# gitAugust/Aruco_Slam

Measured on AMD Instinct MI355X. Metric: frames/s (detect+pose+EKF) at 1280x720, 20 markers, 200 landmarks, higher is better.
Workload: dtype u8/f64; 1 GPU; cfg2: 1280x720 gray stream per GPU, 20 markers/frame in view, 200-landmark EKF (N=603), frames resident in HBM, detector {'polygonalApproxAccuracyRate': 0.03, 'doCornerRefinement': 1}; streams=1, ekf=True, asserted=every frame: 20 markers detected, 20 corrections fused, map_gather=none

## Files before the change

### aruco_slam_amd/csrc/capi.hip

```cpp
#include "common.h"
#include "detect.h"
#include "pose.h"
#include "ekf.h"
#include "win_plan.h"
#include "synth.h"
#include "../../include/aruco_slam_hip.h"
#include <string>
#include <vector>
#include <cfloat>
#include <fstream>
#include <sstream>
#include <cctype>
#include <cstdio>
#include <cstring>
#include <cstdlib>
#include <dlfcn.h>
#include <cstdio>
#include <cmath>
#include <algorithm>
#include <chrono>

using namespace aslam;

namespace {
// ... 117 lines not shown
    bool slam_gate_on = false;
    aslam_gate_params slam_gate_prm{};
    SlamGateArg slam_gate{};
    bool slam_gate_windows = false;
    bool umap_on = false;
    MapCov umap{};
    double* d_map_c = nullptr;
    TrackHealth* h_track_health = nullptr;

    bool win_enabled = true;
    int win_piece = kWinChainFrames;
    bool win_pieces = false;
    unsigned win_epoch = 0;
    bool win_no_early = false;
    bool win_next_split = false;
    struct Pending { bool active = false; int first = 0, count = 0, ev = 0; } pend;
    hipEvent_t ev_obs[2] = {nullptr, nullptr}, ev_idx = nullptr;
    hipStream_t stream_win = nullptr;
    hipEvent_t ev_win[64] = {};
    unsigned win_count = 0;
    unsigned ev_win_next = 0;
    int ev_obs_next = 0;
    bool ev_idx_set = false;
    ObsRaw* h_obs = nullptr;
    unsigned* h_nm = nullptr;
    WinFrame* h_win_frames = nullptr;
    PlanMirror mirror;
    bool mirror_dirty = true;
    int ekf_lo = 0, ekf_hi = 0;
    double last_timing[6] = {0, 0, 0, 0, 0, 0};
// ... 524 lines not shown
    if (c->init.cap_points_per_frame == 0) c->init.cap_points_per_frame = 1u << 19;
    c->max_batch = init->max_batch;
    c->nwaves = init->persistent_waves > 0 ? init->persistent_waves : 4096;
    if (init->persistent_waves <= 0) {
        const char* e = std::getenv("ASLAM_PERSISTENT_WAVES");
        if (e && std::atoi(e) > 0) c->nwaves = std::atoi(e);
    }
    c->sp.Q_k = init->Q_k; c->sp.R_x = init->R_x; c->sp.R_y = init->R_y; c->sp.R_theta = init->R_theta;
    c->sp.kl = init->kl; c->sp.kr = init->kr; c->sp.b = init->b; c->sp.marker_length = init->marker_length;
    c->sp.r2c_tx = init->r2c_t[0]; c->sp.r2c_ty = init->r2c_t[1];
    c->sp.useful_distance_threshold = init->useful_distance_threshold;

    c->win_enabled = std::getenv("ASLAM_NO_WINDOWS") == nullptr;
    c->win_no_early = std::getenv("ASLAM_WIN_NO_EARLY") != nullptr;
    c->win_next_split = std::getenv("ASLAM_WIN_NEXT_SPLIT") != nullptr;
    if (const char* e = std::getenv("ASLAM_WIN_PIECE")) { c->win_piece = std::min(kWinChainFrames, std::max(1, std::atoi(e))); c->win_pieces = true; }
    const int B = c->max_batch;
    const size_t px = (size_t)init->max_rows * init->max_cols;
    const size_t pitch = ((size_t)init->max_cols + 63) / 64 * 64;
    int prio_lo = 0, prio_hi = 0;
    hipDeviceGetStreamPriorityRange(&prio_lo, &prio_hi);
    bool ok = hipStreamCreateWithPriority(&c->stream, hipStreamNonBlocking, prio_lo) == hipSuccess;
    ok = ok && hipStreamCreateWithPriority(&c->stream_ekf, hipStreamNonBlocking, prio_hi) == hipSuccess;
    {
        hipDeviceProp_t prop{};
        const bool known = hipGetDeviceProperties(&prop, init->device_id) == hipSuccess && prop.multiProcessorCount == 256 &&
                           std::strncmp(prop.gcnArchName, "gfx950", 6) == 0;
        const int nxcd = 8, per_xcd = 32;
        const int res = init->ekf_reserved_cus_per_xcd == 0 ? (c->win_enabled ? 4 : 16) : init->ekf_reserved_cus_per_xcd;
        if (known && res > 0 && res < per_xcd) {
// ... 221 lines not shown
int win_steps(const aslam_ctx* c, int first_slot, int K) {
    int n = 0;
    for (int k = 0; k < K; k++) n += 1 + c->h_win_frames[first_slot + k].m;
    return n;
}

void enqueue_window_one(aslam_ctx* c, const WinOp& o, const WinDesc& wd) {
    hipStream_t sa = c->stream_ekf;
    WinDesc cw = wd;
    cw.first_slot = o.frame; cw.K = o.K; cw.piece = 0; cw.log0 = 0; cw.last = 1; cw.mu_out = 0;
    if (++c->win_epoch == 0) c->win_epoch = 1;
    cw.epoch = c->win_epoch;
    cw.nsteps = win_steps(c, o.frame, o.K);
    prof_begin(c, P_EKF_WIN_CHAIN, sa);
    const bool gated = gated_windows(c);
    launch_ekf_win_one(sa, c->ekf, c->sp, cw, c->d_obs, c->d_enc, gated ? &c->slam_gate : nullptr);
    prof_end(c);
    if (gated) {
        prof_begin(c, P_EKF_WIN_GATE_FINISH, sa);
        launch_ekf_win_gate_finish(sa, c->ekf, cw, c->slam_gate, c->d_obs);
        prof_end(c);
    }
}

int enqueue_window_pieces(aslam_ctx* c, const WinOp& o, const WinDesc& wd, hipEvent_t ev_prev_flush) {
    hipStream_t sa = c->stream_ekf;
    struct Piece { WinDesc sub; int nsteps; };
    std::vector<Piece> pieces;
    int log0 = 0, k0 = 0;
    for (int kn : win_piece_sizes(o.K, c->win_piece)) {
        Piece pc;
// ... 2643 lines not shown
```

### aruco_slam_amd/csrc/ekf.h

```cpp
#pragma once
#include "common.h"

namespace aslam {

constexpr int kIdTableSize = 1024;

struct PopRec {
    int id, index, action, det;
    double z[3];
    double r[3];
};
struct LastObs {
    int id, pad;
    double z[3];
};
struct UpdRec {
    int li, pad;
    double Gxm[18];
    double ze[3];
    double r[3];
};
struct MapRecord {
    int id, index;
    double x, y, theta;
// ... 220 lines not shown
    size_t stride;
    const int* robot_of_slot;
    RelocParams prm;
    const ObsRaw* obs;
    const unsigned* n_markers;
    int first, apply;
    RelocRecord* out;
    SlamRelocSeat* seat;
};
hipError_t slam_reloc_alloc(SlamRelocBufs& B, int slots);
void slam_reloc_free(SlamRelocBufs& B);
void launch_slam_reloc_solve(hipStream_t st, const SlamReloc& A, int count);
void launch_slam_reloc_seat(hipStream_t st, const SlamReloc& A, int count);
inline int ekf_win_tiles(int nS) { return nS <= 20 ? 4 : nS <= 41 ? 8 : 12; }
void launch_ekf_win_one(hipStream_t st, const EkfState& E, const SlamParams& sp, const WinDesc& wd, const ObsRaw* obs, const double* enc,
                        const SlamGateArg* gate = nullptr);
void launch_ekf_win_gate_finish(hipStream_t st, const EkfState& E, const WinDesc& wd, const SlamGateArg& gate, const ObsRaw* obs);
void launch_ekf_win_step(hipStream_t st, const EkfState& E, const SlamParams& sp, const WinDesc& wd, const ObsRaw* obs, const double* enc,
                         int s_piece, int s_log0, int s_nsteps, int q_piece, int q_log0, int q_nsteps);
void launch_ekf_win_gather(hipStream_t st, const EkfState& E, const WinDesc& wd);
void launch_ekf_win_next(hipStream_t st, const EkfState& E, const WinDesc& pv, const WinDesc& nx, bool split);
void launch_ekf_win_flush(hipStream_t st, const EkfState& E, const WinDesc& wd);

}
```

### aruco_slam_amd/csrc/ekf_window.hip

```cpp
#include "common.h"
#include "ekf.h"
#include "ekf_dev.h"
#include "ekf_slam_gate.h"
#include <cmath>
#include <cstdlib>
#include <algorithm>

namespace aslam {

constexpr int WBW = 8;
constexpr int kWinPubEvery = 4, kWinPubLag = 4;
#if defined(__HIP__)
constexpr unsigned long long kWinSpinTicks = 2000000;
#else
constexpr unsigned long long kWinSpinTicks = 6000000000ull;
#endif
__device__ __forceinline__ void win_fail(const EkfState& E, unsigned code) { atomicCAS(E.d_win_err, 0u, code); }
template <int NC> __device__ __forceinline__ void win_vmcnt_lag() {
    static_assert(kWinPubLag == 4 && NC >= 1 && NC <= 3, "the counts below are (3 NC + 1) kWinPubLag");
    static_assert((3 * NC + 1) * kWinPubLag <= 63, "vmcnt has six bits");
    if constexpr (NC == 1) ASLAM_VMCNT(16);
    else if constexpr (NC == 2) ASLAM_VMCNT(28);
    else ASLAM_VMCNT(40);
}

#ifdef ASLAM_WIN_STAMPS
#define WSTAMP(i) do { const long long t_ = clock64(); stamp_acc[i] += t_ - stamp_last; stamp_last = t_; } while (0)
#else
#define WSTAMP(i) do { } while (0)
#endif

__host__ __device__ inline int win_log_stride(int T) { return 3 * 16 * T + kWinHdr; }
__host__ __device__ inline int win_tlog_stride(int T) { return 8 * 16 * T; }
enum { WH_TYPE = 0, WH_POS = 1, WH_SI = 2, WH_ZE = 11, WH_C = 14, WH_S = 15, WH_G02 = 16, WH_G12 = 17, WH_A = 18, WH_B = 19, WH_D2 = 20, WH_ACC = 21 };
struct WinGate { static constexpr bool kOn = true; double gate_d2; };
template <class G> struct WinArg : WinDesc, G {};
static_assert(sizeof(WinArg<NoSlamGate>) == sizeof(WinDesc), "the ungated window argument is the window descriptor alone");
__host__ __device__ inline size_t wsm_P(int SPm, int par) { return (size_t)par * SPm * SPm; }
__host__ __device__ inline size_t wsm_LAM(int SPm, int par) { return (size_t)(2 + par) * SPm * SPm; }
__host__ __device__ inline size_t wsm_PSI(int SPm, int par) { return (size_t)(4 + par) * SPm * SPm; }
__host__ __device__ inline size_t wsm_psi(int SPm, int par) { return (size_t)6 * SPm * SPm + (size_t)par * SPm; }
__host__ __device__ inline size_t wsm_MU(int SPm, int par) { return (size_t)6 * SPm * SPm + (size_t)(2 + par) * SPm; }
__host__ __device__ inline size_t wsm_doubles(int SPm) { return (size_t)6 * SPm * SPm + (size_t)4 * SPm; }

// ... 55 lines not shown
        LastObs lo;
        lo.id = o.id; lo.pad = 0;
        const double nanv = __builtin_nan("");
        lo.z[0] = upd ? o.x : nanv; lo.z[1] = upd ? o.y : nanv; lo.z[2] = upd ? o.th : nanv;
        E.d_last[lane] = lo;
    }
    if (lane == 0) { *E.d_nlast = npop; *E.d_npop = npop; *E.d_m = fm; }
}

template <int T, bool ONE> struct WinChainLds {
    static constexpr int SP = 16 * T, SPP = SP + 16, KMAX = ONE ? kWinFrames : kWinPieceMax, NSMAX = KMAX * 64;
    double sA[2][4][SPP];
    double sB[2][4][SPP];
    double sPub[2][3][SPP];
    double sHdr[2][kWinHdr];
    double sRec[2][5][64];
#ifdef ASLAM_WIN_POSE_CHECK
    double sDbg[2][3][SPP];
#endif
    double sMu[SPP];
    int sS[SP];
    int sOff[KMAX + 1];
    unsigned char sPos[NSMAX], sIdx[NSMAX];
    unsigned char sDet[NSMAX];
    static constexpr int kGrown = 2 * 5 * 64 * (int)sizeof(double) - NSMAX;
};
template <bool GATED, class LDS> __device__ __forceinline__ double win_header_entry(const LDS& L, int j, int cb, int fpar, int lane) {
    double v = L.sHdr[cb][lane];
    const int pos = L.sPos[j];
    if (pos != 255) {
        const int a = L.sIdx[j];
        const int q = lane >= WH_ZE && lane < WH_ZE + 3 ? lane - WH_ZE : lane == WH_G02 ? 3 : lane == WH_G12 ? 4 : -1;
        if (q >= 0) v = L.sRec[fpar][q][a];
        if (!GATED && lane == WH_TYPE) v = 1.0;
        if (lane == WH_POS) v = (double)pos;
    }
    return v;
}
template <int T, int RW, bool ONE, class G>
__device__ void win_chain_role(const EkfState& E, const SlamParams& sp, const WinDesc& wd, const G& gate, const ObsRaw* __restrict__ obs,
                               const double* __restrict__ enc, unsigned char* smem) {
    static_assert(ONE || !G::kOn, "only the one-launch window is gated");
    constexpr int SP = 16 * T, SPP = SP + 16, NC = SP / 64;
    constexpr int NWK = (T + RW - 1) / RW, NT = (NWK + (ONE ? 2 : 1)) * 64;
    WinChainLds<T, ONE>& L = *reinterpret_cast<WinChainLds<T, ONE>*>(smem);
    auto& sA = L.sA; auto& sB = L.sB; auto& sPub = L.sPub; auto& sMu = L.sMu; auto& sS = L.sS; auto& sOff = L.sOff;
    auto& sPos = L.sPos; auto& sIdx = L.sIdx; auto& sDet = L.sDet;
    if (threadIdx.x >= NT) return;
    const int tid = threadIdx.x;
    const int nS = wd.nS, s = 3 + 3 * nS;
    const int ld = E.ld;
    const WinFrame* __restrict__ frames = E.d_win_frames;

    const int wave = tid >> 6, lane = tid & 63;
    const int li = lane & 15, lk = lane >> 4;
    for (int e = tid; e < SP; e += NT) sS[e] = e < s ? win_state_index(wd, e) : 0;
    for (int e = tid; e < 2 * 4 * SPP; e += NT) { (&sA[0][0][0])[e] = 0.0; (&sB[0][0][0])[e] = 0.0; }
// ... 139 lines not shown
            printf("worker %d T %d steps %d: barrier-wait %lld | B reads %lld A reads + products%s %lld publish %lld cycles per step\n", wave, T, NS, stamp_acc[0] / (NS + 1),
                   stamp_acc[1] / (NS + 1), ONE ? "" : " + log", stamp_acc[2] / (NS + 1), stamp_acc[3] / (NS + 1));
#endif
        double* Pout = E.d_win_small + wsm_P(E.win_sp_max, wd.wpar);
#pragma unroll
        for (int rr = 0; rr < RW; rr++)
#pragma unroll
            for (int t = 0; t < T; t++)
#pragma unroll
                for (int reg = 0; reg < 4; reg++)
                    if (T % RW == 0 || wave * RW + rr < T) Pout[(size_t)(16 * (wave * RW + rr) + lk + 4 * reg) * SP + 16 * t + li] = acc[rr][t][reg];
        return;
    }

    if (ONE && wave == NWK + 1) {
        ASLAM_LDS_BARRIER();
        win_last_frame(E, frames[wd.first_slot + wd.K - 1], obs + (size_t)(wd.first_slot + wd.K - 1) * kMarkerMax, sOff[wd.K] - sOff[wd.K - 1] - 1, lane);
#ifdef ASLAM_WIN_STAMPS
        long long stamp_acc[2] = {0, 0}, stamp_last = clock64();
#endif
        int fpar = 1;
        for (int j = -1; j < NS; j++) {
            WSTAMP(0);
            if (j > kWinPubLag && j % kWinPubEvery == 0 && lane == 0) win_signal(E.d_win_sync, wd.epoch, j - kWinPubLag);
            if (j >= 0) {
                const int cb = j & 1;
                double* const log = logbase + (size_t)j * win_log_stride(T);
#pragma unroll
                for (int k = 0; k < 3; k++)
#pragma unroll
                    for (int c = 0; c < NC; c++) st_wt(log + k * SP + lane + 64 * c, sA[cb][k][lane + 64 * c]);
                if (sPos[j] == 255) fpar ^= 1;
                if (lane < kWinHdr) st_wt(log + 3 * SP + lane, win_header_entry<G::kOn>(L, j, cb, fpar, lane));
                if ((j + 1) % kWinPubEvery == 0) win_vmcnt_lag<NC>();
            }
            WSTAMP(1);
            ASLAM_LDS_BARRIER();
        }
        ASLAM_VMCNT(0);
        if (lane == 0) win_signal(E.d_win_sync, wd.epoch, NS);
#ifdef ASLAM_WIN_STAMPS
        if (lane == 0) printf("logger T %d steps %d: barrier-wait %lld work %lld cycles per step\n", T, NS, stamp_acc[0] / (NS + 1), stamp_acc[1] / (NS + 1));
#endif
        return;
    }

#ifndef ASLAM_NO_SETPRIO
    __builtin_amdgcn_s_setprio(3);
#endif
    const double kl = sp.kl, kr = sp.kr, inv2b = 1.0 / (2 * sp.b), invb = 1 / sp.b, Qk = sp.Q_k;
    double* const muimg = E.d_win_small + wsm_MU(E.win_sp_max, wd.wpar);
    double mu[NC], pB[4][NC];
    double rp[3][NC];
#pragma unroll
    for (int c = 0; c < NC; c++) {
        const int col = lane + 64 * c;
        mu[c] = col >= s ? 0.0 : from_img ? muimg[col] : E.d_mu[sS[col]];
#pragma unroll
        for (int k = 0; k < 4; k++) pB[k][c] = 0.0;
#pragma unroll
        for (int q = 0; q < 3; q++) rp[q][c] = from_img ? Pimg[(size_t)q * SP + col] : col < s ? E.d_sigma[(size_t)sS[col] * ld + sS[q]] : 0.0;
    }
#ifdef ASLAM_WIN_POSE_CHECK
    double dmax = 0.0, dend = 0.0;
#endif
    double rze0 = 0, rze1 = 0, rze2 = 0, rR0 = 0, rR1 = 0, rR2 = 0, rg02 = 0, rg12 = 0;
    double cth = 1.0, sth = 0.0;
    int fk = -1, fm = 0, fa = 0, vpos = 0;
    bool prev_predict = false;
    bool dirty0 = false, dirty1 = false;
    ObsRaw nObs{};
    if (lane < sOff[1] - 1) nObs = obs[(size_t)wd.first_slot * kMarkerMax + sDet[1 + lane]];
    double e_wl, e_wr, e_dt;
    { const double* e = enc + (size_t)3 * wd.first_slot; e_wl = e[0]; e_wr = e[1]; e_dt = e[2]; }
    ASLAM_LDS_BARRIER();
#ifdef ASLAM_WIN_STAMPS
    long long stamp_acc[11] = {0, 0, 0, 0, 0, 0, 0, 0, 0, 0, 0}, stamp_last = clock64();
    int n_pred = 0;
#endif
    for (int j = -1; j < NS; j++) {
        const int n = j + 1;
        WSTAMP(0);
        if (n < NS) {
            const int nb = n & 1, pb = j & 1;
            const bool is_predict = fa == fm;
// ... 32 lines not shown
                    for (int c = 0; c < NC; c++) {
                        r[0][c] = fma(f[kk][0], pB[kk][c], r[0][c]); r[1][c] = fma(f[kk][1], pB[kk][c], r[1][c]); r[2][c] = fma(f[kk][2], pB[kk][c], r[2][c]);
                        r[3][c] = fma(f[kk][3], pB[kk][c], r[3][c]); r[4][c] = fma(f[kk][4], pB[kk][c], r[4][c]); r[5][c] = fma(f[kk][5], pB[kk][c], r[5][c]);
                    }
                }
            }
#pragma unroll
            for (int c = 0; c < NC; c++) { rp[0][c] = r[0][c]; rp[1][c] = r[1][c]; rp[2][c] = r[2][c]; }
            WSTAMP(1);
            double* const hdr = L.sHdr[nb];
            double A[4][NC], B[4][NC];
            if (is_predict) {
#ifdef ASLAM_WIN_STAMPS
                n_pred++;
#endif
                const int k = ++fk;
                const int slot = wd.first_slot + k;
                fm = ASLAM_WAVE_BCAST(sOff[k + 1] - sOff[k] - 1, 0); fa = 0;
                const double delta_sl = kl * (e_dt * e_wl), delta_sr = kr * (e_dt * e_wr);
                const double delta_theta = (delta_sr - delta_sl) * inv2b;
                const double delta_s = 0.5 * (delta_sr + delta_sl);
#pragma unroll
                for (int c = 0; c < NC; c++) sMu[lane + 64 * c] = mu[c];
                __builtin_amdgcn_wave_barrier();
                const double m0 = sMu[0], m1 = sMu[1], m2 = sMu[2];
#ifdef ASLAM_WIN_STAMPS
                asm volatile("s_waitcnt lgkmcnt(0)" ::: "memory");
                WSTAMP(8);
#endif
                double th = m2 + delta_theta;
// ... 9 lines not shown
                const double P22 = ASLAM_WAVE_BCAST(r[2][0], 2);
#pragma unroll
                for (int c = 0; c < NC; c++) {
                    const int col = lane + 64 * c;
                    const double u = col == 0 ? ua : col == 1 ? ub : 0.0;
                    const double w0 = col == 0 ? f * cm : col == 1 ? f * sm : col == 2 ? f * invb : 0.0;
                    const double w1 = col == 0 ? f * cm : col == 1 ? f * sm : col == 2 ? f * -invb : 0.0;
                    A[0][c] = u;                       B[0][c] = r[2][c];
                    A[1][c] = fma(P22, u, r[2][c]);    B[1][c] = u;
                    A[2][c] = su0 * w0;                B[2][c] = w0;
                    A[3][c] = su1 * w1;                B[3][c] = w1;
                    sA[nb][3][col] = A[3][c]; sB[nb][3][col] = B[3][c];
                }
                if (nb) dirty1 = true; else dirty0 = true;
                const double np0 = m0 + delta_s * cm, np1 = m1 + delta_s * sm;
                if (lane == 0) mu[0] = np0;
                if (lane == 1) mu[0] = np1;
                if (lane == 2) mu[0] = th;
                if (lane < fm) {
                    vpos = sPos[sOff[k] + 1 + lane];
                    const int q = 3 + 3 * vpos;
                    const double mx = sMu[q], my = sMu[q + 1], mth = sMu[q + 2];
                    const double gdx = mx - np0, gdy = my - np1;
                    double gdth = mth - th;
                    wrap1(gdth);
                    const double zh0 = gdx * cth + gdy * sth, zh1 = -gdx * sth + gdy * cth;
                    double z2 = nObs.th - gdth;
                    wrap1(z2);
                    rze0 = nObs.x - zh0; rze1 = nObs.y - zh1; rze2 = z2;
                    rg02 = -gdx * sth + gdy * cth; rg12 = -gdx * cth - gdy * sth;
                    rR0 = nObs.r[0]; rR1 = nObs.r[1]; rR2 = nObs.r[2];
                    double (&rec)[5][64] = L.sRec[k & 1];
                    rec[0][lane] = rze0; rec[1][lane] = rze1; rec[2][lane] = rze2; rec[3][lane] = rg02; rec[4][lane] = rg12;
                }
                __builtin_amdgcn_wave_barrier();
                WSTAMP(10);
                if constexpr (!ONE) {
                    if (wd.last && k == wd.K - 1) win_last_frame(E, frames[slot], obs + (size_t)slot * kMarkerMax, fm, lane);
                }
                if (k + 1 < wd.K) {
                    const int fmn = sOff[k + 2] - sOff[k + 1] - 1;
                    if (lane < fmn) nObs = obs[(size_t)(slot + 1) * kMarkerMax + sDet[sOff[k + 1] + 1 + lane]];
                    const double* e = enc + (size_t)3 * (slot + 1);
                    e_wl = e[0]; e_wr = e[1]; e_dt = e[2];
                }
                if (lane == 0) { hdr[WH_TYPE] = 0.0; hdr[WH_POS] = -1.0; hdr[WH_A] = ua; hdr[WH_B] = ub; hdr[WH_C] = cth; hdr[WH_S] = sth; }
                WSTAMP(2);
            } else {
// ... 23 lines not shown
                Sm[0] += R0; Sm[4] += R1; Sm[8] += R2;
                inv3_fast(Sm, Si);
                double d2 = 0.0;
                bool rejected = false;
                if constexpr (G::kOn) {
                    d2 = slam_gate_d2(Si, ze0, ze1, ze2);
                    rejected = gate.gate_d2 < HUGE_VAL && !(d2 <= gate.gate_d2);
                }
                WSTAMP(4);
#pragma unroll
                for (int c = 0; c < NC; c++) {
                    const double k0 = cc[0][c] * Si[0] + cc[1][c] * Si[3] + cc[2][c] * Si[6];
                    const double k1 = cc[0][c] * Si[1] + cc[1][c] * Si[4] + cc[2][c] * Si[7];
                    const double k2 = cc[0][c] * Si[2] + cc[1][c] * Si[5] + cc[2][c] * Si[8];
                    if constexpr (G::kOn) {
                        const double dm = k0 * ze0 + k1 * ze1 + k2 * ze2;
                        mu[c] = rejected ? mu[c] : mu[c] + dm;
                        A[0][c] = rejected ? 0.0 : -k0; A[1][c] = rejected ? 0.0 : -k1; A[2][c] = rejected ? 0.0 : -k2; A[3][c] = 0.0;
                    } else {
                        mu[c] += k0 * ze0 + k1 * ze1 + k2 * ze2;
                        A[0][c] = -k0; A[1][c] = -k1; A[2][c] = -k2; A[3][c] = 0.0;
                    }
                    B[0][c] = cc[0][c]; B[1][c] = cc[1][c]; B[2][c] = cc[2][c]; B[3][c] = 0.0;
                }
                if (nb ? dirty1 : dirty0) {
#pragma unroll
                    for (int c = 0; c < NC; c++) { sA[nb][3][lane + 64 * c] = 0.0; sB[nb][3][lane + 64 * c] = 0.0; }
                    if (nb) dirty1 = false; else dirty0 = false;
                }
                if (lane == 0) {
#pragma unroll
                    for (int q = 0; q < 9; q++) hdr[WH_SI + q] = Si[q];
                    if constexpr (G::kOn) { hdr[WH_TYPE] = rejected ? 2.0 : 1.0; hdr[WH_D2] = d2; hdr[WH_ACC] = rejected ? 0.0 : 1.0; }
                }
                WSTAMP(5);
            }
#pragma unroll
            for (int c = 0; c < NC; c++) {
                const int col = lane + 64 * c;
                sA[nb][0][col] = A[0][c]; sA[nb][1][col] = A[1][c]; sA[nb][2][col] = A[2][c];
                if (is_predict) { sB[nb][0][col] = B[0][c]; sB[nb][1][col] = B[1][c]; sB[nb][2][col] = B[2][c]; }
#pragma unroll
                for (int kk = 0; kk < 4; kk++) pB[kk][c] = B[kk][c];
            }
            prev_predict = is_predict;
            WSTAMP(6);
        }
        ASLAM_LDS_BARRIER();
    }
#ifdef ASLAM_WIN_STAMPS
    if (lane == 0 && (ONE || wd.piece == 1)) {
        const int nc = NS - n_pred;
        printf("prepare T %d steps %d (%d predict): barrier %lld | rows wait %lld correct %lld | predict path %lld (mean through LDS %lld sincos %lld operands + records %lld global loads, bookkeeping, header %lld) per predict | c %lld S+inv %lld Kt+hdr %lld per correction | operands+log %lld per step\n",
               T, NS, n_pred, stamp_acc[0] / (NS + 1), stamp_acc[7] / NS, stamp_acc[1] / NS, (stamp_acc[2] + stamp_acc[8] + stamp_acc[9] + stamp_acc[10]) / (n_pred ? n_pred : 1), stamp_acc[8] / (n_pred ? n_pred : 1),
               stamp_acc[9] / (n_pred ? n_pred : 1), stamp_acc[10] / (n_pred ? n_pred : 1), stamp_acc[2] / (n_pred ? n_pred : 1), stamp_acc[3] / (nc ? nc : 1), stamp_acc[4] / (nc ? nc : 1),
               stamp_acc[5] / (nc ? nc : 1), stamp_acc[6] / NS);
    }
#endif
#ifdef ASLAM_WIN_POSE_CHECK
    if (lane == 0) printf("pose-check T %d piece %d steps %d: max |prepare - accumulator| pose rows %.3e over the piece, %.3e at its end\n", T, wd.piece, NS, dmax, dend);
#endif
#pragma unroll
    for (int c = 0; c < NC; c++) {
        const int col = lane + 64 * c;
        if (col < s) { muimg[col] = mu[c]; if (wd.mu_out) E.d_mu[sS[col]] = mu[c]; }
    }
}

struct WinReplay { int piece, log0, nsteps, wpar; };
template <int T> struct WinScanLds {
    static constexpr int SP = 16 * T, REC = 3 * SP + kWinHdr;
    double sLam[SP][WBW + 1];
    double sRec[2][REC];
    double sT[2][4][WBW];
};
template <int T, bool ONE, bool GATED>
__device__ void win_scan_role(const EkfState& E, const WinReplay& wd, int b, unsigned epoch, int* sAvail, unsigned char* smem) {
    constexpr int SP = 16 * T, EPT = SP * WBW / 256, REC = 3 * SP + kWinHdr;
    constexpr int RPT = (REC + 191) / 192;
    WinScanLds<T>& L = *reinterpret_cast<WinScanLds<T>*>(smem);
// ... 183 lines not shown
            for (int reg = 0; reg < 4; reg++) Psi[(size_t)(16 * tr + lk + 4 * reg) * SP + 16 * tc + li] = acc[q][reg];
        }
    }
}

__device__ __forceinline__ int win_ticket(unsigned long long* w, unsigned epoch) {
    unsigned long long old = __hip_atomic_load((aslam_gu64*)w, __ATOMIC_RELAXED, __HIP_MEMORY_SCOPE_AGENT);
    for (;;) {
        const bool cur = (unsigned)(old >> 32) == epoch;
        const unsigned long long nw = cur ? old + 1 : ((unsigned long long)epoch << 32) | 1u;
        const unsigned long long prev = atomicCAS(w, old, nw);
        if (prev == old) return cur ? (int)(unsigned)old : 0;
        old = prev;
    }
}
template <int T, int RW, bool ONE, class G = NoSlamGate>
__global__ __launch_bounds__(((T + RW - 1) / RW + (ONE ? 2 : 1)) * 64 > 256 ? ((T + RW - 1) / RW + (ONE ? 2 : 1)) * 64 : 256)
void k_ekf_win_step(EkfState E, SlamParams sp, WinArg<G> wa, WinReplay rs, WinReplay rq, const ObsRaw* __restrict__ obs, const double* __restrict__ enc) {
    const WinDesc& wd = wa;
    constexpr size_t kLds = sizeof(WinChainLds<T, ONE>) > sizeof(WinScanLds<T>) ? sizeof(WinChainLds<T, ONE>) : sizeof(WinScanLds<T>);
    __shared__ __align__(16) unsigned char smem[kLds];
    __shared__ int sTicket, sAvail;
    constexpr int NSCAN = 16 * T / WBW;
    int bx = blockIdx.x;
    if constexpr (ONE) {
        if (threadIdx.x == 0) sTicket = win_ticket(E.d_win_sync + (size_t)kWinSyncLine * (kWinSyncCounters - 1), wd.epoch);
        __syncthreads();
        bx = sTicket;
    }
    if (bx == 0) { if (wd.K > 0) win_chain_role<T, RW, ONE, G>(E, sp, wd, static_cast<const G&>(wa), obs, enc, smem); }
    else if (bx <= NSCAN) { if (rs.nsteps > 0) win_scan_role<T, ONE, G::kOn>(E, rs, bx - 1, wd.epoch, &sAvail, smem); }
    else if (rq.nsteps > 0) win_psi_role<T, ONE, G::kOn>(E, rq, bx - 1 - NSCAN, wd.epoch, &sAvail);
}

constexpr int kWinFinishThreads = 1024;
__global__ __launch_bounds__(kWinFinishThreads) void k_ekf_win_gate_finish(EkfState E, WinDesc wd, GateState gs, const ObsRaw* __restrict__ obs) {
    constexpr int NW = kWinFinishThreads / 64;
    __shared__ double sD2[NW][64];
    __shared__ int sKind[NW][64], sFlag[NW][64], sId[NW][64];
    __shared__ int sOff[kWinFrames + 1], sAtt[kWinFrames], sAcc[kWinFrames];
    const int tid = threadIdx.x, wave = tid >> 6, lane = tid & 63;
    const int K = min(wd.K, kWinFrames);
    const WinFrame* __restrict__ frames = E.d_win_frames + wd.first_slot;
    const int ls = win_log_stride(wd.T), SP = 16 * wd.T;
    const double* __restrict__ hdr0 = E.d_win_log + (size_t)wd.log0 * ls + 3 * SP;
// ... 274 lines not shown
        for (int pc = 0; pc < SPp; pc += 64) {
            double bv[16];
#pragma unroll
            for (int g = 0; g < 16; g++) bv[g] = W[(size_t)(pc + 4 * g) * ld];
#pragma unroll
            for (int g = 0; g < 16; g++) acc = __builtin_amdgcn_mfma_f64_16x16x4f64(-sTt[pc + 4 * g + lk][li], pr == -1 ? bv[g] : 0.0, acc, 0, 0, 0);
        }
#pragma unroll
        for (int reg = 0; reg < 4; reg++) {
            const int c = c0 + lk + 4 * reg;
            if (pr == -1 && sPa[c] == -1) Pout[(size_t)r * SPn + c] = acc[reg];
        }
    }
}

template <int T, bool ONE, class K, class W> static void launch_step_kernel(K kernel, hipStream_t st, int nb, int nt, size_t static_lds, const EkfState& E, const SlamParams& sp,
                                                const W& wd, const WinReplay& rs, const WinReplay& rq, const ObsRaw* obs, const double* enc) {
    static const bool share = std::getenv("ASLAM_WIN_SHARE_CU") != nullptr;
    constexpr size_t cap = (size_t)24 * 1024 + WinChainLds<T, ONE>::kGrown;
    const size_t dyn = share ? 0 : (size_t)84 * 1024 - std::min(static_lds, cap);
    static bool attr_done = false;
    if (!attr_done && dyn > 0) {
        (void)hipFuncSetAttribute(reinterpret_cast<const void*>(kernel), hipFuncAttributeMaxDynamicSharedMemorySize, (int)dyn);
        attr_done = true;
    }
    hipLaunchKernelGGL(kernel, dim3(nb), dim3(nt), dyn, st, E, sp, wd, rs, rq, obs, enc);
}
void launch_ekf_win_step(hipStream_t st, const EkfState& E, const SlamParams& sp, const WinDesc& wd, const ObsRaw* obs, const double* enc,
                         int s_piece, int s_log0, int s_nsteps, int q_piece, int q_log0, int q_nsteps) {
    const WinReplay rs{s_piece, s_log0, s_nsteps, wd.wpar}, rq{q_piece, q_log0, q_nsteps, wd.wpar};
    const int nb = 1 + 16 * wd.T / WBW + wd.T;
    const WinArg<NoSlamGate> wa{wd, {}};
    if (wd.T == 4) launch_step_kernel<4, false>(k_ekf_win_step<4, 2, false>, st, nb, 256, sizeof(WinChainLds<4, false>), E, sp, wa, rs, rq, obs, enc);
    else if (wd.T == 8) launch_step_kernel<8, false>(k_ekf_win_step<8, 2, false>, st, nb, 320, sizeof(WinChainLds<8, false>), E, sp, wa, rs, rq, obs, enc);
    else launch_step_kernel<12, false>(k_ekf_win_step<12, 2, false>, st, nb, 448, sizeof(WinChainLds<12, false>), E, sp, wa, rs, rq, obs, enc);
}
void launch_ekf_win_one(hipStream_t st, const EkfState& E, const SlamParams& sp, const WinDesc& wd, const ObsRaw* obs, const double* enc, const SlamGateArg* gate) {
    const WinReplay r{0, 0, wd.nsteps, wd.wpar};
    const int nb = 1 + 16 * wd.T / WBW + wd.T;
    if (gate) {
        const WinArg<WinGate> wa{wd, WinGate{gate->g.gate_d2}};
        if (wd.T == 4) launch_step_kernel<4, true>(k_ekf_win_step<4, 2, true, WinGate>, st, nb, 256, sizeof(WinChainLds<4, true>), E, sp, wa, r, r, obs, enc);
        else if (wd.T == 8) launch_step_kernel<8, true>(k_ekf_win_step<8, 2, true, WinGate>, st, nb, 384, sizeof(WinChainLds<8, true>), E, sp, wa, r, r, obs, enc);
        else launch_step_kernel<12, true>(k_ekf_win_step<12, 2, true, WinGate>, st, nb, 512, sizeof(WinChainLds<12, true>), E, sp, wa, r, r, obs, enc);
        return;
    }
    const WinArg<NoSlamGate> wa{wd, {}};
    if (wd.T == 4) launch_step_kernel<4, true>(k_ekf_win_step<4, 2, true>, st, nb, 256, sizeof(WinChainLds<4, true>), E, sp, wa, r, r, obs, enc);
    else if (wd.T == 8) launch_step_kernel<8, true>(k_ekf_win_step<8, 2, true>, st, nb, 384, sizeof(WinChainLds<8, true>), E, sp, wa, r, r, obs, enc);
    else launch_step_kernel<12, true>(k_ekf_win_step<12, 2, true>, st, nb, 512, sizeof(WinChainLds<12, true>), E, sp, wa, r, r, obs, enc);
}
void launch_ekf_win_gate_finish(hipStream_t st, const EkfState& E, const WinDesc& wd, const SlamGateArg& gate, const ObsRaw* obs) {
    hipLaunchKernelGGL(k_ekf_win_gate_finish, dim3(1), dim3(kWinFinishThreads), 0, st, E, wd, gate.g, obs);
}
void launch_ekf_win_gather(hipStream_t st, const EkfState& E, const WinDesc& wd) {
    hipLaunchKernelGGL(k_ekf_win_gather, dim3((E.ld + 255) / 256, 16), dim3(256), 0, st, E, wd);
}
static void launch_thin(hipStream_t st, const EkfState& E, const WinDesc& wd, int ncols) {
    const int SP = 16 * wd.T, nb = (ncols + 63) / 64;
    if (wd.T == 4) hipLaunchKernelGGL(k_ekf_win_thin<4>, dim3(nb, 2 * SP / 64), dim3(256), 0, st, E, wd);
    else if (wd.T == 8) hipLaunchKernelGGL(k_ekf_win_thin<8>, dim3(nb, 2 * SP / 64), dim3(256), 0, st, E, wd);
    else hipLaunchKernelGGL(k_ekf_win_thin<12>, dim3(nb, 2 * SP / 64), dim3(256), 0, st, E, wd);
}
void launch_ekf_win_next(hipStream_t st, const EkfState& E, const WinDesc& pv, const WinDesc& nx, bool split) {
    if (!split) {
// ... 27 lines not shown
```

Before: 49300 frames/s.

## Offload S-inverse header and mean update from chain wave to logger wave

The one-launch EKF window kernel's logger wave now recomputes the innovation covariance inverse for the log header and accumulates the state-mean update itself. The serial chain wave stops writing Si to the header and stops updating mu per correction, reloading mu from LDS before each predict step instead. This moves work off the critical serial chain onto an otherwise idle wave, at the cost of extra LDS records (R values, mu and pose buffers) and duplicated inverse arithmetic. An env knob selects which parts are offloaded, and both are on by default.

Result: faster. 50770 frames/s (median of 6 runs) (+3.0%).

```diff
diff --git a/aruco_slam_amd/csrc/capi.hip b/aruco_slam_amd/csrc/capi.hip
--- a/aruco_slam_amd/csrc/capi.hip
+++ b/aruco_slam_amd/csrc/capi.hip
@@ -155,6 +155,7 @@
     unsigned win_epoch = 0;
     bool win_no_early = false;
     bool win_next_split = false;
+    int win_logger_parts = 3;
     struct Pending { bool active = false; int first = 0, count = 0, ev = 0; } pend;
     hipEvent_t ev_obs[2] = {nullptr, nullptr}, ev_idx = nullptr;
     hipStream_t stream_win = nullptr;
@@ -709,6 +710,7 @@
     c->win_enabled = std::getenv("ASLAM_NO_WINDOWS") == nullptr;
     c->win_no_early = std::getenv("ASLAM_WIN_NO_EARLY") != nullptr;
     c->win_next_split = std::getenv("ASLAM_WIN_NEXT_SPLIT") != nullptr;
+    if (const char* e = std::getenv("ASLAM_WIN_LOGGER_PARTS")) c->win_logger_parts = std::atoi(e) & 3;
     if (const char* e = std::getenv("ASLAM_WIN_PIECE")) { c->win_piece = std::min(kWinChainFrames, std::max(1, std::atoi(e))); c->win_pieces = true; }
     const int B = c->max_batch;
     const size_t px = (size_t)init->max_rows * init->max_cols;
@@ -960,7 +962,7 @@
     cw.nsteps = win_steps(c, o.frame, o.K);
     prof_begin(c, P_EKF_WIN_CHAIN, sa);
     const bool gated = gated_windows(c);
-    launch_ekf_win_one(sa, c->ekf, c->sp, cw, c->d_obs, c->d_enc, gated ? &c->slam_gate : nullptr);
+    launch_ekf_win_one(sa, c->ekf, c->sp, cw, c->d_obs, c->d_enc, gated ? &c->slam_gate : nullptr, c->win_logger_parts);
     prof_end(c);
     if (gated) {
         prof_begin(c, P_EKF_WIN_GATE_FINISH, sa);
diff --git a/aruco_slam_amd/csrc/ekf.h b/aruco_slam_amd/csrc/ekf.h
--- a/aruco_slam_amd/csrc/ekf.h
+++ b/aruco_slam_amd/csrc/ekf.h
@@ -258,7 +258,7 @@
 void launch_slam_reloc_seat(hipStream_t st, const SlamReloc& A, int count);
 inline int ekf_win_tiles(int nS) { return nS <= 20 ? 4 : nS <= 41 ? 8 : 12; }
 void launch_ekf_win_one(hipStream_t st, const EkfState& E, const SlamParams& sp, const WinDesc& wd, const ObsRaw* obs, const double* enc,
-                        const SlamGateArg* gate = nullptr);
+                        const SlamGateArg* gate = nullptr, int logger_parts = 3);
 void launch_ekf_win_gate_finish(hipStream_t st, const EkfState& E, const WinDesc& wd, const SlamGateArg& gate, const ObsRaw* obs);
 void launch_ekf_win_step(hipStream_t st, const EkfState& E, const SlamParams& sp, const WinDesc& wd, const ObsRaw* obs, const double* enc,
                          int s_piece, int s_log0, int s_nsteps, int q_piece, int q_log0, int q_nsteps);
diff --git a/aruco_slam_amd/csrc/ekf_window.hip b/aruco_slam_amd/csrc/ekf_window.hip
--- a/aruco_slam_amd/csrc/ekf_window.hip
+++ b/aruco_slam_amd/csrc/ekf_window.hip
@@ -26,8 +26,12 @@
 
 #ifdef ASLAM_WIN_STAMPS
 #define WSTAMP(i) do { const long long t_ = clock64(); stamp_acc[i] += t_ - stamp_last; stamp_last = t_; } while (0)
+#define WSTAMP_AFTER(x) asm volatile("" : "+v"(x))
+#define WSTAMP_BEFORE(x) asm volatile("" :: "v"(x))
 #else
 #define WSTAMP(i) do { } while (0)
+#define WSTAMP_AFTER(x) do { } while (0)
+#define WSTAMP_BEFORE(x) do { } while (0)
 #endif
 
 __host__ __device__ inline int win_log_stride(int T) { return 3 * 16 * T + kWinHdr; }
@@ -113,7 +117,10 @@
     double sB[2][4][SPP];
     double sPub[2][3][SPP];
     double sHdr[2][kWinHdr];
-    double sRec[2][5][64];
+    static constexpr int kRecRows = ONE ? 8 : 5;
+    double sRec[2][kRecRows][64];
+    double sMuL[2][ONE ? SPP : 1];
+    double sPose[2][4];
 #ifdef ASLAM_WIN_POSE_CHECK
     double sDbg[2][3][SPP];
 #endif
@@ -122,7 +129,7 @@
     int sOff[KMAX + 1];
     unsigned char sPos[NSMAX], sIdx[NSMAX];
     unsigned char sDet[NSMAX];
-    static constexpr int kGrown = 2 * 5 * 64 * (int)sizeof(double) - NSMAX;
+    static constexpr int kGrown = (int)sizeof(sRec) + (int)sizeof(sMuL) + (int)sizeof(sPose) - NSMAX;
 };
 template <bool GATED, class LDS> __device__ __forceinline__ double win_header_entry(const LDS& L, int j, int cb, int fpar, int lane) {
     double v = L.sHdr[cb][lane];
@@ -136,10 +143,12 @@
     }
     return v;
 }
-template <int T, int RW, bool ONE, class G>
+template <int T, int RW, bool ONE, class G, int LG>
 __device__ void win_chain_role(const EkfState& E, const SlamParams& sp, const WinDesc& wd, const G& gate, const ObsRaw* __restrict__ obs,
                                const double* __restrict__ enc, unsigned char* smem) {
     static_assert(ONE || !G::kOn, "only the one-launch window is gated");
+    static_assert(ONE || LG == 0, "the piece schedule has no logger wave");
+    constexpr bool LSI = (LG & 1) != 0, LMU = (LG & 2) != 0;
     constexpr int SP = 16 * T, SPP = SP + 16, NC = SP / 64;
     constexpr int NWK = (T + RW - 1) / RW, NT = (NWK + (ONE ? 2 : 1)) * 64;
     WinChainLds<T, ONE>& L = *reinterpret_cast<WinChainLds<T, ONE>*>(smem);
@@ -309,33 +318,128 @@
     }
 
     if (ONE && wave == NWK + 1) {
+        double* const muimg = E.d_win_small + wsm_MU(E.win_sp_max, wd.wpar);
+        double lmu[NC];
         ASLAM_LDS_BARRIER();
+        if constexpr (LMU) {
+#pragma unroll
+            for (int c = 0; c < NC; c++) {
+                const int col = lane + 64 * c;
+                lmu[c] = col >= s ? 0.0 : from_img ? muimg[col] : E.d_mu[sS[col]];
+            }
+        }
         win_last_frame(E, frames[wd.first_slot + wd.K - 1], obs + (size_t)(wd.first_slot + wd.K - 1) * kMarkerMax, sOff[wd.K] - sOff[wd.K - 1] - 1, lane);
+        if constexpr (LMU) ASLAM_VMCNT(0);
 #ifdef ASLAM_WIN_STAMPS
-        long long stamp_acc[2] = {0, 0}, stamp_last = clock64();
+        long long stamp_acc[4] = {0, 0, 0, 0}, stamp_last = clock64();
 #endif
         int fpar = 1;
+        double lcth = 1.0, lsth = 0.0;
+        int p_cur = 255, a_cur = 0;
+        int p_n1 = sPos[0], a_n1 = sIdx[0];
+        int p_n2 = sPos[NS > 1 ? 1 : 0];
         for (int j = -1; j < NS; j++) {
             WSTAMP(0);
             if (j > kWinPubLag && j % kWinPubEvery == 0 && lane == 0) win_signal(E.d_win_sync, wd.epoch, j - kWinPubLag);
+            const int p_n3 = sPos[j + 3 < NS ? j + 3 : NS - 1], a_n2 = sIdx[j + 2 < NS ? j + 2 : NS - 1];
             if (j >= 0) {
                 const int cb = j & 1;
                 double* const log = logbase + (size_t)j * win_log_stride(T);
+                const int pos = p_cur, a = a_cur;
+                const bool corr = pos != 255;
+                if (!corr) fpar ^= 1;
+                const int lrow = corr ? 3 + 3 * pos : 0;
+                const auto& rec = L.sRec[fpar];
+                double av[3][NC];
 #pragma unroll
                 for (int k = 0; k < 3; k++)
 #pragma unroll
-                    for (int c = 0; c < NC; c++) st_wt(log + k * SP + lane + 64 * c, sA[cb][k][lane + 64 * c]);
-                if (sPos[j] == 255) fpar ^= 1;
-                if (lane < kWinHdr) st_wt(log + 3 * SP + lane, win_header_entry<G::kOn>(L, j, cb, fpar, lane));
+                    for (int c = 0; c < NC; c++) av[k][c] = sA[cb][k][lane + 64 * c];
+                const int hq = lane >= WH_ZE && lane < WH_ZE + 3 ? lane - WH_ZE : lane == WH_G02 ? 3 : lane == WH_G12 ? 4 : -1;
+                const double hb = L.sHdr[cb][lane < kWinHdr ? lane : 0], hr = rec[hq >= 0 ? hq : 0][a];
+                const double hC = L.sHdr[cb][WH_C], hS = L.sHdr[cb][WH_S], hT = L.sHdr[cb][WH_TYPE];
+                const double pose = L.sPose[fpar][lane < 3 ? lane : 3];
+                double ze0 = rec[0][a], ze1 = rec[1][a], ze2 = rec[2][a];
+                const double g02 = rec[3][a], g12 = rec[4][a];
+                double R0 = 0.0, R1 = 0.0, R2 = 0.0;
+                double cB[3][6];
+                if constexpr (LSI) {
+                    R0 = rec[5][a]; R1 = rec[6][a]; R2 = rec[7][a];
+#pragma unroll
+                    for (int kk = 0; kk < 3; kk++) {
+                        cB[kk][0] = sB[cb][kk][0]; cB[kk][1] = sB[cb][kk][1]; cB[kk][2] = sB[cb][kk][2];
+                        cB[kk][3] = sB[cb][kk][lrow]; cB[kk][4] = sB[cb][kk][lrow + 1]; cB[kk][5] = sB[cb][kk][lrow + 2];
+                    }
+                }
+#pragma unroll
+                for (int k = 0; k < 3; k++)
+#pragma unroll
+                    for (int c = 0; c < NC; c++) st_wt(log + k * SP + lane + 64 * c, av[k][c]);
+                if (!corr) { lcth = hC; lsth = hS; }
+                double hv = hb;
+                if (corr) {
+                    if (hq >= 0) hv = hr;
+                    if (!G::kOn && lane == WH_TYPE) hv = 1.0;
+                    if (lane == WH_POS) hv = (double)pos;
+                }
+                WSTAMP_BEFORE(hv);
+                WSTAMP(1);
+                if constexpr (LSI) {
+                    double cth = lcth, sth = lsth;
+                    WSTAMP_AFTER(cth); WSTAMP_AFTER(sth);
+                    double Sm[9], Si[9];
+#pragma unroll
+                    for (int kk = 0; kk < 3; kk++) {
+                        const double p0 = cB[kk][0], p1 = cB[kk][1], p2 = cB[kk][2];
+                        const double l0 = cB[kk][3], l1 = cB[kk][4], l2 = cB[kk][5];
+                        Sm[kk * 3 + 0] = (-cth * p0 - sth * p1 + g02 * p2) + (cth * l0 + sth * l1);
+                        Sm[kk * 3 + 1] = (sth * p0 - cth * p1 + g12 * p2) + (-sth * l0 + cth * l1);
+                        Sm[kk * 3 + 2] = l2 - p2;
+                    }
+                    Sm[0] += R0; Sm[4] += R1; Sm[8] += R2;
+                    inv3_fast(Sm, Si);
+#pragma unroll
+                    for (int q = 0; q < 9; q++) hv = corr && lane == WH_SI + q ? Si[q] : hv;
+                }
+                WSTAMP_BEFORE(hv);
+                WSTAMP(2);
+                if (lane < kWinHdr) st_wt(log + 3 * SP + lane, hv);
                 if ((j + 1) % kWinPubEvery == 0) win_vmcnt_lag<NC>();
-            }
-            WSTAMP(1);
+                WSTAMP(1);
+                if constexpr (LMU) {
+                    WSTAMP_AFTER(ze0); WSTAMP_AFTER(ze1); WSTAMP_AFTER(ze2);
+                    const bool upd = corr && !(G::kOn && hT == 2.0);
+#pragma unroll
+                    for (int c = 0; c < NC; c++) {
+                        const double k0 = -av[0][c], k1 = -av[1][c], k2 = -av[2][c];
+                        const double dm = k0 * ze0 + k1 * ze1 + k2 * ze2;
+                        lmu[c] = upd ? lmu[c] + dm : lmu[c];
+                    }
+                    if (!corr && lane < 3) lmu[0] = pose;
+                }
+            }
+            if constexpr (LMU) {
+                if (j + 2 < NS && p_n2 == 255) {
+#pragma unroll
+                    for (int c = 0; c < NC; c++) L.sMuL[j & 1][lane + 64 * c] = lmu[c];
+                }
+            }
+            p_cur = p_n1; a_cur = a_n1; p_n1 = p_n2; a_n1 = a_n2; p_n2 = p_n3;
+            WSTAMP(3);
             ASLAM_LDS_BARRIER();
+        }
+        if constexpr (LMU) {
+#pragma unroll
+            for (int c = 0; c < NC; c++) {
+                const int col = lane + 64 * c;
+                if (col < s) { muimg[col] = lmu[c]; if (wd.mu_out) E.d_mu[sS[col]] = lmu[c]; }
+            }
         }
         ASLAM_VMCNT(0);
         if (lane == 0) win_signal(E.d_win_sync, wd.epoch, NS);
 #ifdef ASLAM_WIN_STAMPS
-        if (lane == 0) printf("logger T %d steps %d: barrier-wait %lld work %lld cycles per step\n", T, NS, stamp_acc[0] / (NS + 1), stamp_acc[1] / (NS + 1));
+        if (lane == 0) printf("logger T %d steps %d: barrier-wait %lld copy + header %lld S^-1 %lld mu %lld cycles per step\n", T, NS, stamp_acc[0] / (NS + 1),
+                              stamp_acc[1] / (NS + 1), stamp_acc[2] / (NS + 1), stamp_acc[3] / (NS + 1));
 #endif
         return;
     }
@@ -364,6 +468,12 @@
     int fk = -1, fm = 0, fa = 0, vpos = 0;
     bool prev_predict = false;
     bool dirty0 = false, dirty1 = false;
+    double pn0 = 0.0, pn1 = 0.0, pth = 0.0;
+    bool prev_rejected = false;
+    if constexpr (LMU) {
+#pragma unroll
+        for (int c = 0; c < NC; c++) L.sMuL[0][lane + 64 * c] = mu[c];
+    }
     ObsRaw nObs{};
     if (lane < sOff[1] - 1) nObs = obs[(size_t)wd.first_slot * kMarkerMax + sDet[1 + lane]];
     double e_wl, e_wr, e_dt;
@@ -426,6 +536,24 @@
 #ifdef ASLAM_WIN_STAMPS
                 n_pred++;
 #endif
+                if constexpr (LMU) {
+#pragma unroll
+                    for (int c = 0; c < NC; c++) mu[c] = L.sMuL[nb][lane + 64 * c];
+                    if (j >= 0) {
+                        if (prev_predict) {
+                            if (lane == 0) mu[0] = pn0;
+                            if (lane == 1) mu[0] = pn1;
+                            if (lane == 2) mu[0] = pth;
+                        } else if (!prev_rejected) {
+                            const double ze0 = ASLAM_WAVE_BCAST(rze0, fm - 1), ze1 = ASLAM_WAVE_BCAST(rze1, fm - 1), ze2 = ASLAM_WAVE_BCAST(rze2, fm - 1);
+#pragma unroll
+                            for (int c = 0; c < NC; c++) {
+                                const double k0 = -sA[pb][0][lane + 64 * c], k1 = -sA[pb][1][lane + 64 * c], k2 = -sA[pb][2][lane + 64 * c];
+                                mu[c] += k0 * ze0 + k1 * ze1 + k2 * ze2;
+                            }
+                        }
+                    }
+                }
                 const int k = ++fk;
                 const int slot = wd.first_slot + k;
                 fm = ASLAM_WAVE_BCAST(sOff[k + 1] - sOff[k] - 1, 0); fa = 0;
@@ -465,9 +593,14 @@
                 }
                 if (nb) dirty1 = true; else dirty0 = true;
                 const double np0 = m0 + delta_s * cm, np1 = m1 + delta_s * sm;
-                if (lane == 0) mu[0] = np0;
-                if (lane == 1) mu[0] = np1;
-                if (lane == 2) mu[0] = th;
+                if constexpr (LMU) {
+                    if (lane < 3) L.sPose[k & 1][lane] = lane == 0 ? np0 : lane == 1 ? np1 : th;
+                    pn0 = np0; pn1 = np1; pth = th;
+                } else {
+                    if (lane == 0) mu[0] = np0;
+                    if (lane == 1) mu[0] = np1;
+                    if (lane == 2) mu[0] = th;
+                }
                 if (lane < fm) {
                     vpos = sPos[sOff[k] + 1 + lane];
                     const int q = 3 + 3 * vpos;
@@ -481,8 +614,9 @@
                     rze0 = nObs.x - zh0; rze1 = nObs.y - zh1; rze2 = z2;
                     rg02 = -gdx * sth + gdy * cth; rg12 = -gdx * cth - gdy * sth;
                     rR0 = nObs.r[0]; rR1 = nObs.r[1]; rR2 = nObs.r[2];
-                    double (&rec)[5][64] = L.sRec[k & 1];
+                    auto& rec = L.sRec[k & 1];
                     rec[0][lane] = rze0; rec[1][lane] = rze1; rec[2][lane] = rze2; rec[3][lane] = rg02; rec[4][lane] = rg12;
+                    if constexpr (LSI) { rec[5][lane] = rR0; rec[6][lane] = rR1; rec[7][lane] = rR2; }
                 }
                 __builtin_amdgcn_wave_barrier();
                 WSTAMP(10);
@@ -536,11 +670,13 @@
                     const double k1 = cc[0][c] * Si[1] + cc[1][c] * Si[4] + cc[2][c] * Si[7];
                     const double k2 = cc[0][c] * Si[2] + cc[1][c] * Si[5] + cc[2][c] * Si[8];
                     if constexpr (G::kOn) {
-                        const double dm = k0 * ze0 + k1 * ze1 + k2 * ze2;
-                        mu[c] = rejected ? mu[c] : mu[c] + dm;
+                        if constexpr (!LMU) {
+                            const double dm = k0 * ze0 + k1 * ze1 + k2 * ze2;
+                            mu[c] = rejected ? mu[c] : mu[c] + dm;
+                        }
                         A[0][c] = rejected ? 0.0 : -k0; A[1][c] = rejected ? 0.0 : -k1; A[2][c] = rejected ? 0.0 : -k2; A[3][c] = 0.0;
                     } else {
-                        mu[c] += k0 * ze0 + k1 * ze1 + k2 * ze2;
+                        if constexpr (!LMU) mu[c] += k0 * ze0 + k1 * ze1 + k2 * ze2;
                         A[0][c] = -k0; A[1][c] = -k1; A[2][c] = -k2; A[3][c] = 0.0;
                     }
                     B[0][c] = cc[0][c]; B[1][c] = cc[1][c]; B[2][c] = cc[2][c]; B[3][c] = 0.0;
@@ -551,10 +687,13 @@
                     if (nb) dirty1 = false; else dirty0 = false;
                 }
                 if (lane == 0) {
-#pragma unroll
-                    for (int q = 0; q < 9; q++) hdr[WH_SI + q] = Si[q];
+                    if constexpr (!LSI) {
+#pragma unroll
+                        for (int q = 0; q < 9; q++) hdr[WH_SI + q] = Si[q];
+                    }
                     if constexpr (G::kOn) { hdr[WH_TYPE] = rejected ? 2.0 : 1.0; hdr[WH_D2] = d2; hdr[WH_ACC] = rejected ? 0.0 : 1.0; }
                 }
+                prev_rejected = rejected;
                 WSTAMP(5);
             }
 #pragma unroll
@@ -582,10 +721,12 @@
 #ifdef ASLAM_WIN_POSE_CHECK
     if (lane == 0) printf("pose-check T %d piece %d steps %d: max |prepare - accumulator| pose rows %.3e over the piece, %.3e at its end\n", T, wd.piece, NS, dmax, dend);
 #endif
-#pragma unroll
-    for (int c = 0; c < NC; c++) {
-        const int col = lane + 64 * c;
-        if (col < s) { muimg[col] = mu[c]; if (wd.mu_out) E.d_mu[sS[col]] = mu[c]; }
+    if constexpr (!LMU) {
+#pragma unroll
+        for (int c = 0; c < NC; c++) {
+            const int col = lane + 64 * c;
+            if (col < s) { muimg[col] = mu[c]; if (wd.mu_out) E.d_mu[sS[col]] = mu[c]; }
+        }
     }
 }
 
@@ -799,7 +940,7 @@
         old = prev;
     }
 }
-template <int T, int RW, bool ONE, class G = NoSlamGate>
+template <int T, int RW, bool ONE, class G = NoSlamGate, int LG = 0>
 __global__ __launch_bounds__(((T + RW - 1) / RW + (ONE ? 2 : 1)) * 64 > 256 ? ((T + RW - 1) / RW + (ONE ? 2 : 1)) * 64 : 256)
 void k_ekf_win_step(EkfState E, SlamParams sp, WinArg<G> wa, WinReplay rs, WinReplay rq, const ObsRaw* __restrict__ obs, const double* __restrict__ enc) {
     const WinDesc& wd = wa;
@@ -813,7 +954,7 @@
         __syncthreads();
         bx = sTicket;
     }
-    if (bx == 0) { if (wd.K > 0) win_chain_role<T, RW, ONE, G>(E, sp, wd, static_cast<const G&>(wa), obs, enc, smem); }
+    if (bx == 0) { if (wd.K > 0) win_chain_role<T, RW, ONE, G, LG>(E, sp, wd, static_cast<const G&>(wa), obs, enc, smem); }
     else if (bx <= NSCAN) { if (rs.nsteps > 0) win_scan_role<T, ONE, G::kOn>(E, rs, bx - 1, wd.epoch, &sAvail, smem); }
     else if (rq.nsteps > 0) win_psi_role<T, ONE, G::kOn>(E, rq, bx - 1 - NSCAN, wd.epoch, &sAvail);
 }
@@ -1118,7 +1259,7 @@
     }
 }
 
-template <int T, bool ONE, class K, class W> static void launch_step_kernel(K kernel, hipStream_t st, int nb, int nt, size_t static_lds, const EkfState& E, const SlamParams& sp,
+template <int T, bool ONE, int LG = 0, class K, class W> static void launch_step_kernel(K kernel, hipStream_t st, int nb, int nt, size_t static_lds, const EkfState& E, const SlamParams& sp,
                                                 const W& wd, const WinReplay& rs, const WinReplay& rq, const ObsRaw* obs, const double* enc) {
     static const bool share = std::getenv("ASLAM_WIN_SHARE_CU") != nullptr;
     constexpr size_t cap = (size_t)24 * 1024 + WinChainLds<T, ONE>::kGrown;
@@ -1139,20 +1280,29 @@
     else if (wd.T == 8) launch_step_kernel<8, false>(k_ekf_win_step<8, 2, false>, st, nb, 320, sizeof(WinChainLds<8, false>), E, sp, wa, rs, rq, obs, enc);
     else launch_step_kernel<12, false>(k_ekf_win_step<12, 2, false>, st, nb, 448, sizeof(WinChainLds<12, false>), E, sp, wa, rs, rq, obs, enc);
 }
-void launch_ekf_win_one(hipStream_t st, const EkfState& E, const SlamParams& sp, const WinDesc& wd, const ObsRaw* obs, const double* enc, const SlamGateArg* gate) {
+template <int T, int NT, class G, class W> static void launch_win_one_lg(hipStream_t st, int nb, int lg, const EkfState& E, const SlamParams& sp, const W& wa, const WinReplay& r,
+                                                                          const ObsRaw* obs, const double* enc) {
+    constexpr size_t lds = sizeof(WinChainLds<T, true>);
+    if (lg == 3) launch_step_kernel<T, true, 3>(k_ekf_win_step<T, 2, true, G, 3>, st, nb, NT, lds, E, sp, wa, r, r, obs, enc);
+    else if (lg == 2) launch_step_kernel<T, true, 2>(k_ekf_win_step<T, 2, true, G, 2>, st, nb, NT, lds, E, sp, wa, r, r, obs, enc);
+    else if (lg == 1) launch_step_kernel<T, true, 1>(k_ekf_win_step<T, 2, true, G, 1>, st, nb, NT, lds, E, sp, wa, r, r, obs, enc);
+    else launch_step_kernel<T, true, 0>(k_ekf_win_step<T, 2, true, G, 0>, st, nb, NT, lds, E, sp, wa, r, r, obs, enc);
+}
+void launch_ekf_win_one(hipStream_t st, const EkfState& E, const SlamParams& sp, const WinDesc& wd, const ObsRaw* obs, const double* enc, const SlamGateArg* gate,
+                        int logger_parts) {
     const WinReplay r{0, 0, wd.nsteps, wd.wpar};
     const int nb = 1 + 16 * wd.T / WBW + wd.T;
     if (gate) {
         const WinArg<WinGate> wa{wd, WinGate{gate->g.gate_d2}};
-        if (wd.T == 4) launch_step_kernel<4, true>(k_ekf_win_step<4, 2, true, WinGate>, st, nb, 256, sizeof(WinChainLds<4, true>), E, sp, wa, r, r, obs, enc);
-        else if (wd.T == 8) launch_step_kernel<8, true>(k_ekf_win_step<8, 2, true, WinGate>, st, nb, 384, sizeof(WinChainLds<8, true>), E, sp, wa, r, r, obs, enc);
-        else launch_step_kernel<12, true>(k_ekf_win_step<12, 2, true, WinGate>, st, nb, 512, sizeof(WinChainLds<12, true>), E, sp, wa, r, r, obs, enc);
+        if (wd.T == 4) launch_win_one_lg<4, 256, WinGate>(st, nb, logger_parts, E, sp, wa, r, obs, enc);
+        else if (wd.T == 8) launch_win_one_lg<8, 384, WinGate>(st, nb, logger_parts, E, sp, wa, r, obs, enc);
+        else launch_win_one_lg<12, 512, WinGate>(st, nb, logger_parts, E, sp, wa, r, obs, enc);
         return;
     }
     const WinArg<NoSlamGate> wa{wd, {}};
-    if (wd.T == 4) launch_step_kernel<4, true>(k_ekf_win_step<4, 2, true>, st, nb, 256, sizeof(WinChainLds<4, true>), E, sp, wa, r, r, obs, enc);
-    else if (wd.T == 8) launch_step_kernel<8, true>(k_ekf_win_step<8, 2, true>, st, nb, 384, sizeof(WinChainLds<8, true>), E, sp, wa, r, r, obs, enc);
-    else launch_step_kernel<12, true>(k_ekf_win_step<12, 2, true>, st, nb, 512, sizeof(WinChainLds<12, true>), E, sp, wa, r, r, obs, enc);
+    if (wd.T == 4) launch_win_one_lg<4, 256, NoSlamGate>(st, nb, logger_parts, E, sp, wa, r, obs, enc);
+    else if (wd.T == 8) launch_win_one_lg<8, 384, NoSlamGate>(st, nb, logger_parts, E, sp, wa, r, obs, enc);
+    else launch_win_one_lg<12, 512, NoSlamGate>(st, nb, logger_parts, E, sp, wa, r, obs, enc);
 }
 void launch_ekf_win_gate_finish(hipStream_t st, const EkfState& E, const WinDesc& wd, const SlamGateArg& gate, const ObsRaw* obs) {
     hipLaunchKernelGGL(k_ekf_win_gate_finish, dim3(1), dim3(kWinFinishThreads), 0, st, E, wd, gate.g, obs);
```
